# nianticlabs/mickey

Hardware: AMD Instinct MI355X
Metric: image pairs/sec (540x720) (higher is better)
Workload: dtype bf16

## Files before the change

include/mickey_hip.h:

```cpp
#ifndef MICKEY_HIP_H
#define MICKEY_HIP_H

#ifdef __cplusplus
extern "C" {
#endif

typedef void* mk_stream_t;

enum { MK_OK = 0, MK_ERR_INVALID_ARGUMENT = 1, MK_ERR_LAUNCH = 2 };
enum { MK_BF16 = 0, MK_F16 = 1, MK_F32 = 2 };
enum { MK_ACT_NONE = 0, MK_ACT_RELU = 1, MK_ACT_GELU = 2 };
enum { MK_EPI_STORE = 0, MK_EPI_LS_RESIDUAL = 1, MK_EPI_QKV = 2, MK_EPI_PATCH = 3 };

int mk_version(void);
const char* mk_last_error(void);


int mk_preprocess_u8(const unsigned char* src, long long stride_img, int n, int Hs, int Ws, float* dst, int H, int W,
                     mk_stream_t stream);


int mk_gemm(const void* A, int lda, const void* W, int ldw, const float* bias, void* out, int ldc, int M, int N, int K,
            int act, int out_is_f32, int dtype, mk_stream_t stream);

// ... 76 lines not shown
int mk_absmax_scale(const float* x, int d0, int d1, int d2, int d3, long long s0, long long s1, long long s2, long long s3,
                    float* work, float* scale, mk_stream_t stream);

long long mk_conv_train_lead_rows(int Wd);
long long mk_conv_train_plane_rows(int nimg, int H, int Wd);
int mk_conv_train_planes(const float* src, long long stride_b, long long stride_c, long long stride_h, long long stride_w, int nimg,
                         int C, int H, int Wd, const float* scale, void* hi, void* lo, int ld, mk_stream_t stream);

int mk_conv_train_weight_planes(const float* w, int Cout, int Cin, int transposed, const float* w_scale, const float* act_scale,
                                void* planes, float* acc_scale, mk_stream_t stream);

long long mk_conv_wgrad_work_floats(int Cout, int Cin, int nimg, int H, int Wd);
int mk_conv_wgrad(const void* gy_hi, const void* gy_lo, int ldg, const void* x_hi, const void* x_lo, int Cout, int Cin, int nimg, int H,
                  int Wd, const float* gy_scale, const float* x_scale, float* work, float* dw, mk_stream_t stream);

int mk_posenc_add(const void* x, const float* pe, float* xs, void* cat, int ld_cat, int groups, int nimg, int npix, int C,
                  int dtype, mk_stream_t stream);

long long mk_linattn_work_floats(int groups, int nimg, int L, int C);
int mk_linattn_kv(const float* qkv, float* kv, float* work, int groups, int nimg, int L, int C, mk_stream_t stream);
int mk_linattn_apply(const float* qkv, const float* kv, void* out, int ldo, int groups, int nimg, int L, int C, int dtype,
                     mk_stream_t stream);

long long mk_linattn_train_work_floats(int nimg, int L, int S, int C);
int mk_linattn_train_fwd(const float* q, long long ldq, long long sq, const float* k, long long ldk, long long sk, const float* v,
                         long long ldv, long long sv, float eps, float* out, float* kv, float* work, int nimg, int L, int S, int C,
                         mk_stream_t stream);
int mk_linattn_train_bwd(const float* q, long long ldq, long long sq, const float* k, long long ldk, long long sk, const float* v,
                         long long ldv, long long sv, const float* kv, const float* go, float eps, float* work, float* gkv, float* gq,
                         float* gk, float* gv, int nimg, int L, int S, int C, mk_stream_t stream);

int mk_head_tails(const float* feat_det, const float* w_score, const float* feat_off, const float* w_xy,
                  const float* feat_depth, const float* w_depth, const float* feat_dsc, float* scr, float* kps, float* depth,
                  float* dsc, int nimg, int h, int w, int C, int Cd, int border, int use_softmax, int use_depth_sigmoid,
                  float max_depth, int norm_dsc, float down, mk_stream_t stream);


long long mk_dual_softmax_work_floats(int B, int n0, int n1, int own_copy);
int mk_dual_softmax(const float* dsc0, const float* dsc1, const float* scr0, const float* scr1, float inv_temperature,
                    int use_dustbin, float dustbin, float* scores, float* kp_scores, float* final_scores, float* work, int B,
                    int C, int n0, int n1, mk_stream_t stream);

long long mk_dual_softmax_split_work_floats(int B, int n0, int n1);
int mk_dual_softmax_split(const float* dsc0, const float* dsc1, const float* scr0, const float* scr1, float inv_temperature,
                          int use_dustbin, float dustbin, float* scores, float* kp_scores, float* final_scores, float* work,
                          int B, int C, int n0, int n1, mk_stream_t stream);
// ... 87 lines not shown
```

mickey_amd/_native.py:

```python
import ctypes
import os

import torch

from . import build as _build

MK_BF16, MK_F16, MK_F32 = 0, 1, 2
ACT_NONE, ACT_RELU, ACT_GELU = 0, 1, 2

_P, _I, _L, _F, _U = ctypes.c_void_p, ctypes.c_int, ctypes.c_longlong, ctypes.c_float, ctypes.c_ulonglong
_CODES = {"p": _P, "i": _I, "l": _L, "f": _F, "u": _U}

SIGNATURES = {
    "mk_version": ("i", ""),
    "mk_last_error": ("s", ""),
    "mk_preprocess_u8": ("i", "pliiipiip"),
    "mk_gemm": ("i", "pipippiiiiiiip"),
    "mk_gemm_grouped": ("i", "pilpilplpiliiiiiiip"),
    "mk_gemm_ls_residual": ("i", "pipipppiiiiip"),
    "mk_gemm_qkv": ("i", "pipippppiiiifip"),
    "mk_gemm_patch_embed": ("i", "pipipppiiiiip"),
    "mk_gemm_ls_residual_ln": ("i", "pipippppipppiiiiip"),
    "mk_gemm_patch_embed_ln": ("i", "pipipppppiiiiip"),
    "mk_cls_token_ln": ("i", "pppppiiiip"),
# ... 5 lines not shown
    "mk_layernorm": ("i", "pippfpiipiiiiiiiiiip"),
    "mk_layernorm_nchw": ("i", "pippfpiiiiiip"),
    "mk_gemm_ln128": ("i", "pilpilppfpipiiiiiiip"),
    "mk_layernorm_planes": ("i", "pippfppifpiiiiiiiiipp"),
    "mk_flash_attn_fwd": ("i", "ppppiiiiiip"),
    "mk_bordered_rows": ("l", "iii"),
    "mk_conv3x3": ("i", "pliplipilplplpiliiiiiiip"),
    "mk_conv3x3_split": ("i", "pplipplipilplppiliiiiiiffpp"),
    "mk_conv3x3_split_dscale": ("i", "ppipipiiiipp"),
    "mk_split_planes": ("i", "plilfpplpp"),
    "mk_absmax_scale_work_floats": ("l", ""),
    "mk_absmax_scale": ("i", "piiiillllppp"),
    "mk_conv_train_lead_rows": ("l", "i"),
    "mk_conv_train_plane_rows": ("l", "iii"),
    "mk_conv_train_planes": ("i", "plllliiiipppip"),
    "mk_conv_train_weight_planes": ("i", "piiippppp"),
    "mk_conv_wgrad_work_floats": ("l", "iiiii"),
    "mk_conv_wgrad": ("i", "ppippiiiiippppp"),
    "mk_gemm_grouped_split": ("i", "ppilpilplppiliiiiiffpp"),
    "mk_posenc_add": ("i", "ppppiiiiiip"),
    "mk_linattn_work_floats": ("l", "iiii"),
    "mk_linattn_kv": ("i", "pppiiiip"),
    "mk_linattn_apply": ("i", "pppiiiiiip"),
    "mk_linattn_train_work_floats": ("l", "iiii"),
    "mk_linattn_train_fwd": ("i", "pllpllpllfpppiiiip"),
    "mk_linattn_train_bwd": ("i", "pllpllpllppfpppppiiiip"),
    "mk_head_tails": ("i", "pppppppppppiiiiiiiififp"),
    "mk_dual_softmax_work_floats": ("l", "iiii"),
    "mk_dual_softmax": ("i", "ppppfifppppiiiip"),
    "mk_dual_softmax_split_work_floats": ("l", "iii"),
    "mk_dual_softmax_split": ("i", "ppppfifppppiiiip"),
    "mk_sinkhorn_work_floats": ("l", "iii"),
    "mk_sinkhorn": ("i", "ppppfippppiiiip"),
    "mk_dual_softmax_kf": ("i", "ppppfifppppiiiipip"),
    "mk_dual_softmax_split_kf": ("i", "ppppfifppppiiiipip"),
    "mk_sinkhorn_kf": ("i", "ppppfippppiiiipip"),
    "mk_mutual_nn": ("i", "ppppiiip"),
    "mk_dual_softmax_train_work_floats": ("l", "iiii"),
    "mk_dual_softmax_train": ("i", "ppppfppppppiiiiip"),
    "mk_dual_softmax_bwd_work_floats": ("l", "iiii"),
    "mk_dual_softmax_bwd": ("i", "ppppfpppppppppiiiiip"),
    "mk_exprace_topk_work_bytes": ("l", "iiil"),
    "mk_exprace_topk_state_bytes": ("l", "ii"),
    "mk_exprace_topk": ("i", "ppuupppppiiliip"),
    "mk_counter_add": ("i", "pup"),
    "mk_gather_backproject": ("i", "ppppppppppppiiiiip"),
# ... 95 lines not shown
```

mickey_amd/csrc/mk_heads.hip:

```cpp
#include "mk_common.hpp"

namespace {
using namespace mk;

constexpr int KVW = 272;
constexpr int KV_CHUNK = 64;

template <typename T>
__global__ __launch_bounds__(256) void posenc_kernel(const T* __restrict__ x, const float* __restrict__ pe,
                                                     float* __restrict__ xs, T* __restrict__ cat, int ld_cat, long long rows,
                                                     int npix, int C, long long total4) {
  for (long long i = blockIdx.x * (long long)blockDim.x + threadIdx.x; i < total4; i += (long long)gridDim.x * blockDim.x) {
    const int c4 = (int)(i % (C / 4));
    const long long r = i / (C / 4);
    const long long rr = r % rows;
    const int pix = (int)(rr % npix);
    const typename Lp<T>::V4 v = *(const typename Lp<T>::V4*)(x + r * C + c4 * 4);
    f32x4 f;
#pragma unroll
    for (int e = 0; e < 4; ++e) f[e] = (float)v[e];
    if (pe) f += *(const f32x4*)(pe + (long long)pix * C + c4 * 4);
    *(f32x4*)(xs + r * C + c4 * 4) = f;
    typename Lp<T>::V4 o;
#pragma unroll
    for (int e = 0; e < 4; ++e) o[e] = (T)f[e];
    *(typename Lp<T>::V4*)(cat + r * ld_cat + c4 * 4) = o;
  }
}

__device__ __forceinline__ float phi(float x) { return x > 0.f ? x + 1.0f : expf(x); }

__global__ __launch_bounds__(256) void linattn_kv_partial(const float* __restrict__ qkv, float* __restrict__ part, int L, int C,
                                                          int nchunk) {
  extern __shared__ __attribute__((aligned(16))) float skv[];
  const int H = C >> 4;
  const long long gi = blockIdx.y;
  const int chunk = blockIdx.x;
  const int t = threadIdx.x, lane = t & 63, wave = t >> 6;
  const int s0 = chunk * KV_CHUNK, ntok = min(L, s0 + KV_CHUNK) - s0;
  const float invL = 1.0f / (float)L;
  const float* base = qkv + (gi * (long long)L + s0) * 3 * C + C;
  const int c4 = 2 * C / 4;
  for (int it = 0; it < KV_CHUNK * c4 / 256; ++it) {
    const int i = it * 256 + t;
    const int s = min(i / c4, ntok - 1), c = (i % c4) * 4;
    glds16(base + (long long)s * 3 * C + c, (char*)skv + (it * 256 + wave * 64) * 16);
  }
  asm volatile("s_waitcnt vmcnt(0)" ::: "memory");
  __syncthreads();
  for (int i = t; i < ntok * (C / 4); i += 256) {
    const int s = i / (C / 4), c = (i - s * (C / 4)) * 4;
    f32x4 v = *(const f32x4*)(skv + s * 2 * C + c);
#pragma unroll
    for (int e = 0; e < 4; ++e) v[e] = phi(v[e]);
    *(f32x4*)(skv + s * 2 * C + c) = v;
  }
  __syncthreads();
  const int h = lane >> 3, vh = (lane >> 2) & 1, dg = lane & 3;
  float acc[4][8];
  float ks[4] = {0.f, 0.f, 0.f, 0.f};
#pragma unroll
  for (int a = 0; a < 4; ++a)
#pragma unroll
    for (int e = 0; e < 8; ++e) acc[a][e] = 0.f;
  if (h < H) {
    for (int s = wave; s < ntok; s += 4) {
      const float* row = skv + s * 2 * C + h * 16;
      const f32x4 k4 = *(const f32x4*)(row + dg * 4);
      const f32x4 v0 = *(const f32x4*)(row + C + vh * 8), v1 = *(const f32x4*)(row + C + vh * 8 + 4);
#pragma unroll
      for (int a = 0; a < 4; ++a) {
#pragma unroll
        for (int e = 0; e < 4; ++e) {
          acc[a][e] += k4[a] * (v0[e] * invL);
          acc[a][4 + e] += k4[a] * (v1[e] * invL);
        }
        ks[a] += k4[a];
      }
    }
  }
  __syncthreads();
  if (h < H) {
    float* o = skv + (wave * H + h) * KVW;
#pragma unroll
    for (int a = 0; a < 4; ++a) {
#pragma unroll
      for (int e = 0; e < 8; ++e) o[(dg * 4 + a) * 16 + vh * 8 + e] = acc[a][e];
      if (vh == 0) o[256 + dg * 4 + a] = ks[a];
    }
  }
  __syncthreads();
  for (int i = t; i < H * KVW; i += 256) {
    const int hh = i / KVW, e = i - hh * KVW;
    const float r = ((skv[(0 * H + hh) * KVW + e] + skv[(1 * H + hh) * KVW + e]) + skv[(2 * H + hh) * KVW + e]) + skv[(3 * H + hh) * KVW + e];
    part[(((gi * H + hh) * nchunk) + chunk) * KVW + e] = r;
  }
}

__global__ __launch_bounds__(KVW) void linattn_kv_reduce(const float* __restrict__ part, float* __restrict__ kv, int nchunk) {
  const long long gih = blockIdx.x;
  const int t = threadIdx.x;
// ... 3 lines not shown
}

template <typename T>
__global__ __launch_bounds__(256) void linattn_apply_kernel(const float* __restrict__ qkv, const float* __restrict__ kv,
                                                            T* __restrict__ out, int ldo, int L, int C) {
  extern __shared__ __attribute__((aligned(16))) float skv[];
  const int H = C >> 4;
  const long long gi = blockIdx.y;
  for (int i = threadIdx.x; i < H * KVW; i += blockDim.x) skv[(i / KVW) * 273 + (i % KVW)] = kv[gi * H * KVW + i];
  __syncthreads();
  const int tpb = 256 / H;
  const int h = threadIdx.x % H;
  const int s = blockIdx.x * tpb + threadIdx.x / H;
  if (s >= L || threadIdx.x >= tpb * H) return;
  const float* qrow = qkv + (gi * L + s) * 3 * C + h * 16;
  float Q[16];
#pragma unroll
  for (int d4 = 0; d4 < 4; ++d4) {
    const f32x4 t4 = *(const f32x4*)(qrow + d4 * 4);
#pragma unroll
    for (int e = 0; e < 4; ++e) Q[d4 * 4 + e] = phi(t4[e]);
  }
  const float* K = skv + h * 273;
  float z = 0.f;
#pragma unroll
  for (int d = 0; d < 16; ++d) z += Q[d] * K[256 + d];
  const float scale = (float)L / (z + 1e-6f);
  typename Lp<T>::V8 o0, o1;
#pragma unroll
  for (int v = 0; v < 16; ++v) {
    float a = 0.f;
#pragma unroll
    for (int d = 0; d < 16; ++d) a += Q[d] * K[d * 16 + v];
    a *= scale;
    if (v < 8) o0[v] = (T)a; else o1[v - 8] = (T)a;
  }
  T* orow = out + (gi * L + s) * ldo + h * 16;
  *(typename Lp<T>::V8*)orow = o0;
  *(typename Lp<T>::V8*)(orow + 8) = o1;
}


__global__ __launch_bounds__(256) void kp_depth_tail_kernel(const float* __restrict__ fdet, const float* __restrict__ wsc,
                                                            const float* __restrict__ foff, const float* __restrict__ wxy,
                                                            const float* __restrict__ fdep, const float* __restrict__ wd,
                                                            float* __restrict__ scr, float* __restrict__ kps,
                                                            float* __restrict__ depth, int nimg, int h, int w, int C,
                                                            int use_depth_sigmoid, float max_depth, float down) {
  const int n = h * w;
  const long long gp = blockIdx.x * 4LL + (threadIdx.x >> 6);
  if (gp >= (long long)nimg * n) return;
  const int lane = threadIdx.x & 63;
  const int img = (int)(gp / n), p = (int)(gp % n);
  float as = 0.f, ax = 0.f, ay = 0.f, ad = 0.f;
  for (int c = lane; c < C; c += 64) {
    const float fo = foff[gp * C + c];
    as += fdet[gp * C + c] * wsc[c];
    ax += fo * wxy[c];
    ay += fo * wxy[C + c];
// ... 56 lines not shown

__global__ __launch_bounds__(256) void dsc_tail_kernel(const float* __restrict__ fdsc, float* __restrict__ dsc, int n, int Cd,
                                                       int norm_dsc) {
  extern __shared__ __attribute__((aligned(16))) float tile[];
  const int img = blockIdx.y, p0 = blockIdx.x * 64;
  const int lane = threadIdx.x & 63, wave = threadIdx.x >> 6;
  for (int pp = wave; pp < 64; pp += 4) {
    const int p = p0 + pp;
    if (p >= n) break;
    const float* f = fdsc + ((long long)img * n + p) * Cd;
    float q = 0.f;
    for (int c = lane; c < Cd; c += 64) q += f[c] * f[c];
    q = wave_sum(q);
    const float sc = norm_dsc ? 1.0f / sqrtf(q + 1e-10f) : 1.0f;
    for (int c = lane; c < Cd; c += 64) tile[c * 65 + pp] = f[c] * sc;
  }
  __syncthreads();
  for (int i = threadIdx.x; i < Cd * 64; i += blockDim.x) {
    const int c = i >> 6, pp = i & 63;
    if (p0 + pp < n) dsc[((long long)img * Cd + c) * n + p0 + pp] = tile[c * 65 + pp];
  }
}

template <typename T>
__global__ __launch_bounds__(256, 2) void gemm_ln128_kernel(const T* __restrict__ A, int lda, long long strideA, const T* __restrict__ W,
                                                            int ldw, long long strideW, const float* __restrict__ lnw,
                                                            const float* __restrict__ lnb, float eps, float* __restrict__ resid, int ldr,
                                                            T* __restrict__ out, int ldo, int groups, int M, int K, int bord_h, int bord_w) {
  using V8 = typename Lp<T>::V8;
  using V4 = typename Lp<T>::V4;
  extern __shared__ __attribute__((aligned(16))) char smem[];
  const int lane = threadIdx.x & 63, wave = threadIdx.x >> 6;
  const int g = blockIdx.x % groups, wg = blockIdx.x / groups, nwg = gridDim.x / groups;
  const int ks = K >> 5;
  const T* Wg = W + (long long)g * strideW;
  for (int i = threadIdx.x; i < 128 * ks * 4; i += 256) {
    const int c = i & 3, s = (i >> 2) % ks, n = i / (4 * ks);
    const uint4 v = *(const uint4*)(Wg + (long long)n * ldw + s * 32 + c * 8);
    *(uint4*)(smem + ((s * 128 + n) * 64 + ((c ^ ((n >> 2) & 3)) << 4))) = v;
  }
  float* slw = (float*)(smem + 128 * K * 2);
  float* slb = slw + 128;
  if (threadIdx.x < 128) {
    slw[threadIdx.x] = lnw[g * 128 + threadIdx.x];
    slb[threadIdx.x] = lnb[g * 128 + threadIdx.x];
  }
// ... 19 lines not shown
  };
  if (wg < ntile) {
    load_x(wg);
    if (resid) load_r(wg);
  }
  for (int tile = wg; tile < ntile; tile += nwg) {
    const int row = row_of(tile);
    const bool ok = row < M;
    const bool more = tile + nwg < ntile;
    f32x4 acc[8];
#pragma unroll
    for (int f = 0; f < 8; ++f) acc[f] = f32x4{0.f, 0.f, 0.f, 0.f};
#pragma unroll
    for (int s = 0; s < 8; ++s) {
      if (s >= ks) break;
#pragma unroll
      for (int f = 0; f < 8; ++f) {
        const int n = f * 16 + r16;
        const V8 wf = *(const V8*)(smem + ((s * 128 + n) * 64 + ((q ^ ((n >> 2) & 3)) << 4)));
        acc[f] = Lp<T>::mma16(wf, xf[s], acc[f]);
      }
    }
    if (more) load_x(tile + nwg);
    float sm = 0.f;
#pragma unroll
    for (int f = 0; f < 8; ++f) sm += (acc[f][0] + acc[f][1]) + (acc[f][2] + acc[f][3]);
    sm += __shfl_xor(sm, 16, 64);
    sm += __shfl_xor(sm, 32, 64);
    const float mean = sm * (1.0f / 128.0f);
    float qs = 0.f;
#pragma unroll
    for (int f = 0; f < 8; ++f) {
#pragma unroll
      for (int e = 0; e < 4; ++e) {
        acc[f][e] -= mean;
        qs += acc[f][e] * acc[f][e];
      }
    }
    qs += __shfl_xor(qs, 16, 64);
    qs += __shfl_xor(qs, 32, 64);
    const float rstd = 1.0f / sqrtf(qs * (1.0f / 128.0f) + eps);
    if (ok) {
      const long long grow = (long long)g * M + row;
      const long long orow = bord_h > 0 ? (long long)g * brows + bordered_row(row, bord_h, bord_w) : grow;
#pragma unroll
      for (int f = 0; f < 8; ++f) {
        const int fe = f * 16 + q * 4;
        const f32x4 ww = *(const f32x4*)(slw + fe), bb = *(const f32x4*)(slb + fe);
        f32x4 y;
#pragma unroll
        for (int e = 0; e < 4; ++e) y[e] = acc[f][e] * rstd * ww[e] + bb[e];
        if (resid) {
          y += rv[f];
          *(f32x4*)(resid + grow * ldr + fe) = y;
        }
        V4 o;
#pragma unroll
        for (int e = 0; e < 4; ++e) o[e] = (T)y[e];
        *(V4*)(out + orow * ldo + fe) = o;
      }
    }
    if (resid && more) load_r(tile + nwg);
  }
}

}

extern "C" {

int mk_posenc_add(const void* x, const float* pe, float* xs, void* cat, int ld_cat, int groups, int nimg, int npix, int C,
                  int dtype, mk_stream_t stream) {
  MK_CHECK_ARG(x && xs && cat && groups > 0 && nimg > 0 && npix > 0 && C % 8 == 0 && ld_cat % 4 == 0 && ld_cat >= C,
               "mk_posenc_add: bad args");
  const long long rows = (long long)nimg * npix;
  const long long total4 = (long long)groups * rows * (C / 4);
  int blocks = (int)((total4 + 255) / 256);
  if (blocks > 8192) blocks = 8192;
  if (dtype == MK_BF16)
    hipLaunchKernelGGL(posenc_kernel<__bf16>, dim3(blocks), dim3(256), 0, (hipStream_t)stream, (const __bf16*)x, pe, xs,
                       (__bf16*)cat, ld_cat, rows, npix, C, total4);
  else if (dtype == MK_F16)
    hipLaunchKernelGGL(posenc_kernel<_Float16>, dim3(blocks), dim3(256), 0, (hipStream_t)stream, (const _Float16*)x, pe, xs,
                       (_Float16*)cat, ld_cat, rows, npix, C, total4);
  else
    hipLaunchKernelGGL(posenc_kernel<float>, dim3(blocks), dim3(256), 0, (hipStream_t)stream, (const float*)x, pe, xs,
                       (float*)cat, ld_cat, rows, npix, C, total4);
// ... 16 lines not shown
                     nchunk);
  MK_CHECK_LAUNCH();
  hipLaunchKernelGGL(linattn_kv_reduce, dim3(gih), dim3(KVW), 0, (hipStream_t)stream, work, kv, nchunk);
  MK_CHECK_LAUNCH();
  return MK_OK;
}

int mk_linattn_apply(const float* qkv, const float* kv, void* out, int ldo, int groups, int nimg, int L, int C, int dtype,
                     mk_stream_t stream) {
  const int H = C / 16;
  MK_CHECK_ARG(qkv && kv && out && groups > 0 && nimg > 0 && L > 0 && C % 16 == 0 && H <= 64 && ldo % 8 == 0 && ldo >= C,
               "mk_linattn_apply: bad args");
  const int tpb = 256 / H;
  dim3 grid((L + tpb - 1) / tpb, groups * nimg);
  const size_t lds = (size_t)H * 273 * sizeof(float);
  if (dtype == MK_BF16)
    hipLaunchKernelGGL(linattn_apply_kernel<__bf16>, grid, dim3(256), lds, (hipStream_t)stream, qkv, kv, (__bf16*)out, ldo, L,
                       C);
  else if (dtype == MK_F16)
    hipLaunchKernelGGL(linattn_apply_kernel<_Float16>, grid, dim3(256), lds, (hipStream_t)stream, qkv, kv, (_Float16*)out,
                       ldo, L, C);
  else
    hipLaunchKernelGGL(linattn_apply_kernel<float>, grid, dim3(256), lds, (hipStream_t)stream, qkv, kv, (float*)out, ldo, L, C);
  MK_CHECK_LAUNCH();
  return MK_OK;
}

int mk_gemm_ln128(const void* A, int lda, long long strideA, const void* W, int ldw, long long strideW, const float* ln_w,
                  const float* ln_b, float eps, float* resid, int ldr, void* out, int ldo, int groups, int M, int K, int bord_h,
                  int bord_w, int dtype, mk_stream_t stream) {
  MK_CHECK_ARG(A && W && ln_w && ln_b && out, "mk_gemm_ln128: null pointer");
  MK_CHECK_ARG(dtype == MK_BF16 || dtype == MK_F16, "mk_gemm_ln128: 16-bit operands only");
  MK_CHECK_ARG(groups > 0 && M > 0 && K >= 32 && K <= 256 && K % 32 == 0 && lda % 8 == 0 && lda >= K && ldw % 8 == 0 && ldw >= K &&
                   ldo % 4 == 0 && ldo >= 128 && (!resid || (ldr % 4 == 0 && ldr >= 128)),
               "mk_gemm_ln128: bad geometry (K a multiple of 32 up to 256, 128 output features)");
  MK_CHECK_ARG((((uintptr_t)A | (uintptr_t)W) & 15) == 0 && ((uintptr_t)out & 7) == 0 && (strideA % 8) == 0 && (strideW % 8) == 0,
               "mk_gemm_ln128: operands must be 16-byte aligned");
  MK_CHECK_ARG(bord_h == 0 || (bord_w > 0 && M % (bord_h * bord_w) == 0), "mk_gemm_ln128: bordered output needs M = nimg * bord_h * bord_w");
  const int lds = 128 * K * 2 + 1024;
  const int ntile = (M + 63) / 64;
  int per_group = ((K > 128 ? 2 : 3) * mk::gemm::num_cus() + groups - 1) / groups;
  if (per_group > ntile) per_group = ntile;
  const dim3 grid((unsigned)(per_group * groups));
  hipError_t e = hipSuccess;
  if (dtype == MK_BF16) {
    static bool done = false;
// ... 39 lines not shown
```

mickey_amd/ops.py:

```python

import numpy as np
import torch


from ._native import ACT_GELU, ACT_NONE, ACT_RELU, call, dtype_code, ptr, query, stream

LOG2E = 1.4426950408889634


def _chk(t, dtype=None):
    assert t.is_cuda and t.is_contiguous(), "expected a contiguous device tensor"
    if dtype is not None:
        assert t.dtype == dtype, "expected %s, got %s" % (dtype, t.dtype)
    return t


def preprocess_u8(frames, H, W, out=None):
    assert frames.is_cuda and frames.dtype == torch.uint8 and frames.dim() == 4 and frames.shape[3] == 3 and frames.is_contiguous()
    n, Hs, Ws, _ = frames.shape
    if out is None:
        out = torch.empty((n, 3, H, W), device=frames.device, dtype=torch.float32)
    call("mk_preprocess_u8", ptr(frames), Hs * Ws * 3, n, Hs, Ws, ptr(out), H, W, stream())
    return out

# ... 295 lines not shown
        dw = torch.empty((Cout, Cin, 3, 3), device=xp[0].device, dtype=torch.float32)
    assert dw.dtype == torch.float32 and dw.is_contiguous() and tuple(dw.shape) == (Cout, Cin, 3, 3)
    work = torch.empty(max(1, int(query("mk_conv_wgrad_work_floats", Cout, Cin, nimg, H, W))), device=dw.device, dtype=torch.float32)
    call("mk_conv_wgrad", ptr(gy[0]), ptr(gy[1]), ldg, ptr(xp[0]), ptr(xp[1]), Cout, Cin, nimg, H, W, ptr(gy_scale), ptr(x_scale),
         ptr(work), ptr(dw), stream())
    return dw


def posenc_add(x, pe, xs, cat, groups, nimg, npix, C):
    call("mk_posenc_add", ptr(x), ptr(pe), ptr(xs), ptr(cat), cat.stride(-2), groups, nimg, npix, C, dtype_code(x.dtype),
         stream())


def linattn_work_floats(groups, nimg, L, C):
    return query("mk_linattn_work_floats", groups, nimg, L, C)


def linattn_kv(qkv, kv, work, groups, nimg, L, C):
    call("mk_linattn_kv", ptr(qkv), ptr(kv), ptr(work), groups, nimg, L, C, stream())


def linattn_apply(qkv, kv, out, ldo, groups, nimg, L, C):
    call("mk_linattn_apply", ptr(qkv), ptr(kv), ptr(out), ldo, groups, nimg, L, C, dtype_code(out.dtype), stream())


def _attn_rows(t):
    N, T, H, D = t.shape
    assert t.dtype == torch.float32 and D == 16 and t.stride(3) == 1 and (H == 1 or t.stride(2) == 16)
    ld = t.stride(1) if T > 1 else H * 16
    return ptr(t), ld, t.stride(0) if N > 1 else T * ld


def linattn_train_fwd(q, k, v, eps):
    N, L, H, _ = q.shape
    S, C = k.shape[1], H * 16
    out = torch.empty((N, L, H, 16), device=q.device, dtype=torch.float32)
    kv = torch.empty((N * H, 272), device=q.device, dtype=torch.float32)
    work = torch.empty(int(query("mk_linattn_train_work_floats", N, L, S, C)), device=q.device, dtype=torch.float32)
    call("mk_linattn_train_fwd", *_attn_rows(q), *_attn_rows(k), *_attn_rows(v), float(eps), ptr(out), ptr(kv), ptr(work), N, L, S, C,
         stream())
    return out, kv


def linattn_train_bwd(q, k, v, kv, go, eps, need):
    N, L, H, _ = q.shape
    S, C = k.shape[1], H * 16
# ... 330 lines not shown
```

mickey_amd/pipeline.py:

```python
import torch

from . import ops
from . import weights as wts_mod


class Workspace:

    def __init__(self):
        self.bufs = {}
        self.sat_flag = None

    def get_planes(self, name, shape, device, zero=False):
        t = self.get(name, (2,) + tuple(shape), torch.float16, device, zero=zero)
        return t[0], t[1]

    def get(self, name, shape, dtype, device, zero=False):
        key = (name, tuple(shape), dtype)
        t = self.bufs.get(key)
        if t is None or t.device != device:
            t = (torch.zeros if zero else torch.empty)(tuple(shape), dtype=dtype, device=device)
            self.bufs[key] = t
        return t


# ... 113 lines not shown
                              stride_in1=R * co, stride_in2=s_in, stride_w=rb.w2.shape[1] * rb.w2.shape[2], stride_bias=co,
                              stride_out=(M if last else R) * co, out_bordered=not last)
            if not last:
                xp = xo
        else:
            h1 = ws.get("rb%d_h" % bi + geo, (G, R, co), lp, dev, zero=True)
            xo = ws.get("rb%d_x" % bi + geo, (G, M if last else R, co), lp, dev, zero=not last)
            ops.conv3x3(x_in, c_in, rb.w1, rb.b1, h1, co, G, nimg, gh, gw, act=ops.ACT_RELU, stride_in1=s_in,
                        stride_w=rb.w1.shape[1] * rb.w1.shape[2], stride_bias=co, stride_out=R * co, out_bordered=True)
            ops.conv3x3(h1, co, rb.w2, rb.b2, xo, co, G, nimg, gh, gw, act=ops.ACT_RELU, in2=x_in, C2=c_in,
                        stride_in1=R * co, stride_in2=s_in, stride_w=rb.w2.shape[1] * rb.w2.shape[2], stride_bias=co,
                        stride_out=(M if last else R) * co, out_bordered=not last)
        x_in, c_in, s_in = xo, co, R * co
    C = c_in
    xs = ws.get("att_xs", (G, M, C), torch.float32, dev)
    cat = ws.get("att_cat", (G, M, 2 * C), lp, dev)
    pe = wts_mod.sine_pos_table(W, C, gh, gw, dev)
    kp_pe, dsc_pe = bool(mk["KP_HEADS"]["POS_ENCODING"]), bool(mk["DSC_HEAD"]["POS_ENCODING"])
    if kp_pe == dsc_pe:
        ops.posenc_add(x_in, pe if kp_pe else None, xs, cat, G, nimg, n, C)
    else:
        ops.posenc_add(x_in[:3], pe if kp_pe else None, xs[:3], cat[:3], 3, nimg, n, C)
        ops.posenc_add(x_in[3:], pe if dsc_pe else None, xs[3:], cat[3:], 1, nimg, n, C)
    qkv = ws.get("att_qkv", (G, M, 3 * C), torch.float32, dev)
    kv = ws.get("att_kv", (G * nimg * (C // 16), 272), torch.float32, dev)
    kvw = ws.get("att_kvw", (ops.linattn_work_floats(G, nimg, n, C),), torch.float32, dev)
    msg = ws.get("att_msg", (G, M, C), lp, dev)
    mrg = ws.get("att_mrg", (G, M, C), torch.float32, dev)
    hid = ws.get("att_hid", (G, M, 2 * C), lp, dev)
    if split:
        x4 = None
        x4h, x4l = plane_pair("att_out", (G, R, C))
    else:
        x4 = ws.get("att_out" + geo, (G, R, C), lp, dev, zero=True)
    nl = len(W.att)
    if split:
        catp = ws.get_planes("att_cat_hl", (G, M, 2 * C), dev)
        msgp = ws.get_planes("att_msg_hl", (G, M, C), dev)
        hidp = ws.get_planes("att_hid_hl", (G, M, 2 * C), dev)
    for li, lay in enumerate(W.att):
        last = li == nl - 1
        if split:
            if li == 0:
                ops.split_planes(cat[:, :, :C], catp[0][:, :, :C], catp[1][:, :, :C], sat=sat)
            ops.gemm_grouped_split(catp, lay.qkv_w, None, qkv, G, M, 3 * C, C, 2 * C, 3 * C, M * 2 * C, 3 * C * 2 * C, 0, M * 3 * C,
                                   w_scale=wsc(lay.qkv_w), sat=sat)
            ops.linattn_kv(qkv, kv, kvw, G, nimg, n, C)
            ops.linattn_apply(qkv, kv, msg, C, G, nimg, n, C)
            ops.split_planes(msg, msgp[0], msgp[1], sat=sat)
            ops.gemm_grouped_split(msgp, lay.merge_w, None, mrg, G, M, C, C, C, C, M * C, C * 2 * C, 0, M * C, w_scale=wsc(lay.merge_w), sat=sat)
            ops.layernorm(mrg, lay.n1w, lay.n1b, 1e-5, out=(catp[0][:, :, C:], catp[1][:, :, C:]), ldo=2 * C, rows_out=G * M,
                          rows_per_img=G * M, wgroup_rows=M, sat=sat)
            ops.gemm_grouped_split(catp, lay.mlp0_w, None, hidp, G, M, 2 * C, 2 * C, 2 * C, 2 * C, M * 2 * C, 2 * C * 2 * 2 * C, 0,
                                   M * 2 * C, act=ops.ACT_RELU, w_scale=wsc(lay.mlp0_w), sat=sat)
            ops.gemm_grouped_split(hidp, lay.mlp2_w, None, mrg, G, M, C, 2 * C, 2 * C, C, M * 2 * C, C * 2 * 2 * C, 0, M * C,
                                   w_scale=wsc(lay.mlp2_w), sat=sat)
        else:
            ops.gemm_grouped(cat, lay.qkv_w, None, qkv, G, M, 3 * C, C, 2 * C, C, 3 * C, M * 2 * C, 3 * C * C, 0, M * 3 * C)
            ops.linattn_kv(qkv, kv, kvw, G, nimg, n, C)
            ops.linattn_apply(qkv, kv, msg, C, G, nimg, n, C)
            fused_ln = C == 128 and lp != torch.float32
            if fused_ln:
                ops.gemm_ln128(msg, lay.merge_w, lay.n1w, lay.n1b, 1e-5, cat[:, :, C:], G, M, C, ldo=2 * C)
            else:
                ops.gemm_grouped(msg, lay.merge_w, None, mrg, G, M, C, C, C, C, C, M * C, C * C, 0, M * C)
                ops.layernorm(mrg, lay.n1w, lay.n1b, 1e-5, out=cat[:, :, C:], ldo=2 * C, rows_out=G * M, rows_per_img=G * M,
                              wgroup_rows=M)
            ops.gemm_grouped(cat, lay.mlp0_w, None, hid, G, M, 2 * C, 2 * C, 2 * C, 2 * C, 2 * C, M * 2 * C, 4 * C * C, 0,
                             M * 2 * C, act=ops.ACT_RELU)
            if not fused_ln:
                ops.gemm_grouped(hid, lay.mlp2_w, None, mrg, G, M, C, 2 * C, 2 * C, 2 * C, C, M * 2 * C, 2 * C * C, 0, M * C)
        if split:
            o2 = (x4h, x4l) if last else (catp[0][:, :, :C], catp[1][:, :, :C])
        else:
            o2 = x4 if last else cat
        if not split and C == 128 and lp != torch.float32:
            ops.gemm_ln128(hid, lay.mlp2_w, lay.n2w, lay.n2b, 1e-5, o2, G, M, 2 * C, ldo=C if last else 2 * C, resid=xs,
                           bordered=(nimg, gh, gw) if last else None)
        else:
# ... 104 lines not shown
```

Before: 274.5.

## Fuse QKV projection into linear-attention KV and apply kernels with merge+LayerNorm

Adds two fused kernels for C=128 bf16/f16. One computes the K/V projections with MFMA directly from the concatenated input and accumulates the per-chunk KV outer products. The other recomputes Q, applies attention, then runs the merge GEMM and LayerNorm in the same kernel, writing straight into the concat buffer. This removes the fp32 qkv tensor, the intermediate message buffer and separate launches, at the cost of recomputing projections in both kernels and needing large LDS with more register pressure. It is enabled by default for the non-split low-precision path.

New measurement: 277.4 (median of 6 runs). 1.01x the previous value.

```diff
diff --git a/include/mickey_hip.h b/include/mickey_hip.h
--- a/include/mickey_hip.h
+++ b/include/mickey_hip.h
@@ -122,6 +122,13 @@
 int mk_linattn_apply(const float* qkv, const float* kv, void* out, int ldo, int groups, int nimg, int L, int C, int dtype,
                      mk_stream_t stream);
 
+int mk_linattn_kv_fused(const void* x, int lda, long long strideX, const void* qkv_w, int ldw, long long strideW, float* kv,
+                        float* work, int groups, int nimg, int L, int C, int dtype, mk_stream_t stream);
+int mk_linattn_apply_fused(const void* x, int lda, long long strideX, const void* qkv_w, int ldw, long long strideW, const float* kv,
+                           const void* merge_w, int ldwm, long long strideWm, const float* ln_w, const float* ln_b, float eps,
+                           void* out, int ldo, long long strideOut, int groups, int nimg, int L, int C, int dtype,
+                           mk_stream_t stream);
+
 long long mk_linattn_train_work_floats(int nimg, int L, int S, int C);
 int mk_linattn_train_fwd(const float* q, long long ldq, long long sq, const float* k, long long ldk, long long sk, const float* v,
                          long long ldv, long long sv, float eps, float* out, float* kv, float* work, int nimg, int L, int S, int C,
diff --git a/mickey_amd/_native.py b/mickey_amd/_native.py
--- a/mickey_amd/_native.py
+++ b/mickey_amd/_native.py
@@ -51,6 +51,8 @@
     "mk_linattn_work_floats": ("l", "iiii"),
     "mk_linattn_kv": ("i", "pppiiiip"),
     "mk_linattn_apply": ("i", "pppiiiiiip"),
+    "mk_linattn_kv_fused": ("i", "pilpilppiiiiip"),
+    "mk_linattn_apply_fused": ("i", "pilpilppilppfpiliiiiip"),
     "mk_linattn_train_work_floats": ("l", "iiii"),
     "mk_linattn_train_fwd": ("i", "pllpllpllfpppiiiip"),
     "mk_linattn_train_bwd": ("i", "pllpllpllppfpppppiiiip"),
diff --git a/mickey_amd/csrc/mk_heads.hip b/mickey_amd/csrc/mk_heads.hip
--- a/mickey_amd/csrc/mk_heads.hip
+++ b/mickey_amd/csrc/mk_heads.hip
@@ -29,6 +29,32 @@
 }
 
 __device__ __forceinline__ float phi(float x) { return x > 0.f ? x + 1.0f : expf(x); }
+
+template <int NV>
+__device__ __forceinline__ void kv_outer(float (&acc)[4][NV], float (&ks)[4], const f32x4 k4, const float (&vs)[NV]) {
+#pragma unroll
+  for (int a = 0; a < 4; ++a) {
+#pragma unroll
+    for (int e = 0; e < NV; ++e) acc[a][e] += k4[a] * vs[e];
+    ks[a] += k4[a];
+  }
+}
+
+template <int NV, typename KVAT, typename KSAT, typename PUT>
+__device__ __forceinline__ void linattn_apply_cols(const float (&Q)[16], KVAT kvat, KSAT ksat, const int L, PUT put) {
+  float z = 0.f;
+#pragma unroll
+  for (int d = 0; d < 16; ++d) z += Q[d] * ksat(d);
+  const float scale = (float)L / (z + 1e-6f);
+#pragma unroll
+  for (int v = 0; v < NV; ++v) {
+    float s = 0.f;
+#pragma unroll
+    for (int d = 0; d < 16; ++d) s += Q[d] * kvat(d, v);
+    s *= scale;
+    put(v, s);
+  }
+}
 
 __global__ __launch_bounds__(256) void linattn_kv_partial(const float* __restrict__ qkv, float* __restrict__ part, int L, int C,
                                                           int nchunk) {
@@ -68,15 +94,8 @@
       const float* row = skv + s * 2 * C + h * 16;
       const f32x4 k4 = *(const f32x4*)(row + dg * 4);
       const f32x4 v0 = *(const f32x4*)(row + C + vh * 8), v1 = *(const f32x4*)(row + C + vh * 8 + 4);
-#pragma unroll
-      for (int a = 0; a < 4; ++a) {
-#pragma unroll
-        for (int e = 0; e < 4; ++e) {
-          acc[a][e] += k4[a] * (v0[e] * invL);
-          acc[a][4 + e] += k4[a] * (v1[e] * invL);
-        }
-        ks[a] += k4[a];
-      }
+      const float v8[8] = {v0[0] * invL, v0[1] * invL, v0[2] * invL, v0[3] * invL, v1[0] * invL, v1[1] * invL, v1[2] * invL, v1[3] * invL};
+      kv_outer<8>(acc, ks, k4, v8);
     }
   }
   __syncthreads();
@@ -126,19 +145,9 @@
     for (int e = 0; e < 4; ++e) Q[d4 * 4 + e] = phi(t4[e]);
   }
   const float* K = skv + h * 273;
-  float z = 0.f;
-#pragma unroll
-  for (int d = 0; d < 16; ++d) z += Q[d] * K[256 + d];
-  const float scale = (float)L / (z + 1e-6f);
   typename Lp<T>::V8 o0, o1;
-#pragma unroll
-  for (int v = 0; v < 16; ++v) {
-    float a = 0.f;
-#pragma unroll
-    for (int d = 0; d < 16; ++d) a += Q[d] * K[d * 16 + v];
-    a *= scale;
-    if (v < 8) o0[v] = (T)a; else o1[v - 8] = (T)a;
-  }
+  linattn_apply_cols<16>(Q, [&](int d, int v) { return K[d * 16 + v]; }, [&](int d) { return K[256 + d]; }, L,
+                         [&](int v, float a) { if (v < 8) o0[v] = (T)a; else o1[v - 8] = (T)a; });
   T* orow = out + (gi * L + s) * ldo + h * 16;
   *(typename Lp<T>::V8*)orow = o0;
   *(typename Lp<T>::V8*)(orow + 8) = o1;
@@ -241,6 +250,33 @@
   }
 }
 
+__device__ __forceinline__ float ln128_centre(f32x4 (&acc)[8], const float eps) {
+  float sm = 0.f;
+#pragma unroll
+  for (int f = 0; f < 8; ++f) sm += (acc[f][0] + acc[f][1]) + (acc[f][2] + acc[f][3]);
+  sm += __shfl_xor(sm, 16, 64);
+  sm += __shfl_xor(sm, 32, 64);
+  const float mean = sm * (1.0f / 128.0f);
+  float qs = 0.f;
+#pragma unroll
+  for (int f = 0; f < 8; ++f) {
+#pragma unroll
+    for (int e = 0; e < 4; ++e) {
+      acc[f][e] -= mean;
+      qs += acc[f][e] * acc[f][e];
+    }
+  }
+  qs += __shfl_xor(qs, 16, 64);
+  qs += __shfl_xor(qs, 32, 64);
+  return 1.0f / sqrtf(qs * (1.0f / 128.0f) + eps);
+}
+__device__ __forceinline__ f32x4 ln128_affine(const f32x4 c, const float rstd, const f32x4 ww, const f32x4 bb) {
+  f32x4 y;
+#pragma unroll
+  for (int e = 0; e < 4; ++e) y[e] = c[e] * rstd * ww[e] + bb[e];
+  return y;
+}
+
 template <typename T>
 __global__ __launch_bounds__(256, 2) void gemm_ln128_kernel(const T* __restrict__ A, int lda, long long strideA, const T* __restrict__ W,
                                                             int ldw, long long strideW, const float* __restrict__ lnw,
@@ -306,24 +342,7 @@
       }
     }
     if (more) load_x(tile + nwg);
-    float sm = 0.f;
-#pragma unroll
-    for (int f = 0; f < 8; ++f) sm += (acc[f][0] + acc[f][1]) + (acc[f][2] + acc[f][3]);
-    sm += __shfl_xor(sm, 16, 64);
-    sm += __shfl_xor(sm, 32, 64);
-    const float mean = sm * (1.0f / 128.0f);
-    float qs = 0.f;
-#pragma unroll
-    for (int f = 0; f < 8; ++f) {
-#pragma unroll
-      for (int e = 0; e < 4; ++e) {
-        acc[f][e] -= mean;
-        qs += acc[f][e] * acc[f][e];
-      }
-    }
-    qs += __shfl_xor(qs, 16, 64);
-    qs += __shfl_xor(qs, 32, 64);
-    const float rstd = 1.0f / sqrtf(qs * (1.0f / 128.0f) + eps);
+    const float rstd = ln128_centre(acc, eps);
     if (ok) {
       const long long grow = (long long)g * M + row;
       const long long orow = bord_h > 0 ? (long long)g * brows + bordered_row(row, bord_h, bord_w) : grow;
@@ -331,9 +350,7 @@
       for (int f = 0; f < 8; ++f) {
         const int fe = f * 16 + q * 4;
         const f32x4 ww = *(const f32x4*)(slw + fe), bb = *(const f32x4*)(slb + fe);
-        f32x4 y;
-#pragma unroll
-        for (int e = 0; e < 4; ++e) y[e] = acc[f][e] * rstd * ww[e] + bb[e];
+        f32x4 y = ln128_affine(acc[f], rstd, ww, bb);
         if (resid) {
           y += rv[f];
           *(f32x4*)(resid + grow * ldr + fe) = y;
@@ -346,6 +363,258 @@
     }
     if (resid && more) load_r(tile + nwg);
   }
+}
+
+constexpr int FC = 128;
+
+template <typename T, int ROWS>
+__device__ __forceinline__ void w_rows_to_lds(const T* __restrict__ Wg, const int ldw, char* dst, const int tid, const int nthr) {
+  for (int i = tid; i < ROWS * 16; i += nthr) {
+    const int c = i & 3, st = (i >> 2) & 3, n = i >> 4;
+    const uint4 v = *(const uint4*)(Wg + (long long)n * ldw + st * 32 + c * 8);
+    *(uint4*)(dst + ((st * ROWS + n) * 64 + ((c ^ ((n >> 2) & 3)) << 4))) = v;
+  }
+}
+template <typename T, int ROWS>
+__device__ __forceinline__ typename Lp<T>::V8 w_frag(const char* w, const int st, const int n, const int q) {
+  return *(const typename Lp<T>::V8*)(w + ((st * ROWS + n) * 64 + ((q ^ ((n >> 2) & 3)) << 4)));
+}
+
+template <typename T>
+__global__ __launch_bounds__(256, 2) void linattn_kv_fused_kernel(const T* __restrict__ X, int lda, long long strideX,
+                                                                  const T* __restrict__ Wqkv, int ldw, long long strideW,
+                                                                  float* __restrict__ part, int nimg, int L, int nchunk) {
+  using V8 = typename Lp<T>::V8;
+  __shared__ __attribute__((aligned(16))) float stage[4 * 1024];
+  constexpr int H = FC / 16;
+  const int tid = threadIdx.x, lane = tid & 63, wave = __builtin_amdgcn_readfirstlane(tid >> 6);
+  const long long gi = blockIdx.y;
+  const int g = (int)(gi / nimg), img = (int)(gi % nimg);
+  float* stg = stage + wave * 1024;
+  const int r16 = lane & 15, q = lane >> 4;
+  const int hp = lane >> 5, vg = (lane >> 2) & 7, dg = lane & 3;
+  const float invL = 1.0f / (float)L;
+  V8 wf[4][4];
+  {
+    const T* Wg = Wqkv + (long long)g * strideW + q * 8;
+#pragma unroll
+    for (int j = 0; j < 4; ++j) {
+      const int n = FC + (j >> 1) * FC + wave * 32 + (j & 1) * 16 + r16;
+#pragma unroll
+      for (int st = 0; st < 4; ++st) wf[st][j] = *(const V8*)(Wg + (long long)n * ldw + st * 32);
+    }
+  }
+  const T* xi = X + (long long)g * strideX + (long long)img * L * lda + q * 8;
+  auto load_x = [&](int first, V8(&xf)[4]) {
+    const int s = min(first + 4 * r16, L - 1);
+#pragma unroll
+    for (int st = 0; st < 4; ++st) xf[st] = *(const V8*)(xi + (long long)s * lda + st * 32);
+  };
+  V8 xf[4], xn[4];
+  int chunk = blockIdx.x;
+  if (chunk < nchunk) load_x(chunk * KV_CHUNK, xf);
+  for (; chunk < nchunk; chunk += gridDim.x) {
+    const int ntok = min(L, (chunk + 1) * KV_CHUNK) - chunk * KV_CHUNK;
+    float acc[4][4][2], ks[4][4];
+#pragma unroll
+    for (int b = 0; b < 4; ++b)
+#pragma unroll
+      for (int a = 0; a < 4; ++a) acc[b][a][0] = acc[b][a][1] = ks[b][a] = 0.f;
+#pragma unroll
+    for (int b = 0; b < 4; ++b) {
+      f32x4 kvq[4];
+#pragma unroll
+      for (int j = 0; j < 4; ++j) kvq[j] = f32x4{0.f, 0.f, 0.f, 0.f};
+#pragma unroll
+      for (int st = 0; st < 4; ++st)
+#pragma unroll
+        for (int j = 0; j < 4; ++j) kvq[j] = Lp<T>::mma16(wf[st][j], xf[st], kvq[j]);
+#pragma unroll
+      for (int st = 0; st < 4; ++st) xn[st] = xf[st];
+      if (b < 3) load_x(chunk * KV_CHUNK + b + 1, xn);
+      else if (chunk + (int)gridDim.x < nchunk) load_x((chunk + gridDim.x) * KV_CHUNK, xn);
+#pragma unroll
+      for (int j = 0; j < 2; ++j)
+#pragma unroll
+        for (int e = 0; e < 4; ++e) {
+          kvq[j][e] = phi(kvq[j][e]);
+          kvq[2 + j][e] = kvq[2 + j][e] * invL;
+        }
+#pragma unroll
+      for (int j = 0; j < 4; ++j) *(f32x4*)(stg + r16 * 64 + (((j * 4 + q) ^ r16) << 2)) = kvq[j];
+      __builtin_amdgcn_wave_barrier();
+      auto token = [&](const int t) {
+        const f32x4 k4 = *(const f32x4*)(stg + t * 64 + (((hp * 4 + dg) ^ t) << 2));
+        const float2 v2 = *(const float2*)(stg + t * 64 + (((8 + hp * 4 + (vg >> 1)) ^ t) << 2) + (vg & 1) * 2);
+        const float vs[2] = {v2.x, v2.y};
+        kv_outer<2>(acc[b], ks[b], k4, vs);
+      };
+      if (ntok == KV_CHUNK) {
+#pragma unroll
+        for (int t = 0; t < 16; ++t) token(t);
+      } else {
+#pragma unroll 1
+        for (int t = 0; b + 4 * t < ntok; ++t) token(t);
+      }
+      __builtin_amdgcn_wave_barrier();
+#pragma unroll
+      for (int st = 0; st < 4; ++st) xf[st] = xn[st];
+    }
+    float* o = part + (((gi * H + 2 * wave + hp) * nchunk) + chunk) * KVW;
+#pragma unroll
+    for (int a = 0; a < 4; ++a) {
+      float2 r;
+      r.x = ((acc[0][a][0] + acc[1][a][0]) + acc[2][a][0]) + acc[3][a][0];
+      r.y = ((acc[0][a][1] + acc[1][a][1]) + acc[2][a][1]) + acc[3][a][1];
+      *(float2*)(o + (dg * 4 + a) * 16 + vg * 2) = r;
+    }
+    if (vg == 0) {
+      f32x4 r;
+#pragma unroll
+      for (int a = 0; a < 4; ++a) r[a] = ((ks[0][a] + ks[1][a]) + ks[2][a]) + ks[3][a];
+      *(f32x4*)(o + 256 + dg * 4) = r;
+    }
+  }
+}
+
+template <typename T, bool MERGE>
+__global__ __launch_bounds__(512) void linattn_apply_fused_kernel(const T* X, int lda, long long strideX, const T* __restrict__ Wqkv,
+                                                                  int ldw, long long strideW, const float* __restrict__ kv,
+                                                                  const T* __restrict__ Wm, int ldwm, long long strideWm,
+                                                                  const float* __restrict__ lnw, const float* __restrict__ lnb, float eps,
+                                                                  T* out, int ldo, long long strideO, int nimg, int L) {
+  using V8 = typename Lp<T>::V8;
+  using V4 = typename Lp<T>::V4;
+  extern __shared__ __attribute__((aligned(16))) char smem[];
+  constexpr int H = FC / 16;
+  const int tid = threadIdx.x, lane = tid & 63, wave = __builtin_amdgcn_readfirstlane(tid >> 6);
+  const long long gi = blockIdx.y;
+  const int g = (int)(gi / nimg), img = (int)(gi % nimg);
+  char* swm = smem + FC * FC * 2;
+  float* slw = (float*)(smem + 2 * FC * FC * 2);
+  float* slb = slw + FC;
+  w_rows_to_lds<T, FC>(Wqkv + (long long)g * strideW, ldw, smem, tid, 512);
+  if (MERGE) {
+    w_rows_to_lds<T, FC>(Wm + (long long)g * strideWm, ldwm, swm, tid, 512);
+    if (tid < FC) {
+      slw[tid] = lnw[g * FC + tid];
+      slb[tid] = lnb[g * FC + tid];
+    }
+  }
+  __syncthreads();
+  float* stq = (float*)(smem + 2 * FC * FC * 2 + 1024) + wave * 2048;
+  const int r16 = lane & 15, q = lane >> 4;
+  const int par = lane >> 5, h = (lane >> 2) & 7, vg = lane & 3;
+  f32x4 kreg[16], ksum[4];
+  {
+    const float* kp = kv + (gi * H + h) * KVW;
+#pragma unroll
+    for (int d = 0; d < 16; ++d) kreg[d] = *(const f32x4*)(kp + d * 16 + vg * 4);
+#pragma unroll
+    for (int d4 = 0; d4 < 4; ++d4) ksum[d4] = *(const f32x4*)(kp + 256 + d4 * 4);
+  }
+  const int ntile = (L + 15) >> 4, step = gridDim.x * 8;
+  const T* xi = X + (long long)g * strideX + (long long)img * L * lda + q * 8;
+  T* oi = out + (long long)g * strideO + (long long)img * L * ldo;
+  V8 xf[4];
+  auto load_x = [&](int tile) {
+    const int s = min(tile * 16 + r16, L - 1);
+#pragma unroll
+    for (int st = 0; st < 4; ++st) xf[st] = *(const V8*)(xi + (long long)s * lda + st * 32);
+  };
+  int tile = blockIdx.x * 8 + wave;
+  if (tile < ntile) load_x(tile);
+  for (; tile < ntile; tile += step) {
+    f32x4 acc[8];
+#pragma unroll
+    for (int f = 0; f < 8; ++f) acc[f] = f32x4{0.f, 0.f, 0.f, 0.f};
+#pragma unroll
+    for (int st = 0; st < 4; ++st)
+#pragma unroll
+      for (int f = 0; f < 8; ++f) acc[f] = Lp<T>::mma16(w_frag<T, FC>(smem, st, f * 16 + r16, q), xf[st], acc[f]);
+    if (tile + step < ntile) load_x(tile + step);
+#pragma unroll
+    for (int f = 0; f < 8; ++f) {
+#pragma unroll
+      for (int e = 0; e < 4; ++e) acc[f][e] = phi(acc[f][e]);
+      const int c = f * 4 + q;
+      *(f32x4*)(stq + r16 * 128 + ((c ^ r16 ^ ((c >> 4) << 1)) << 2)) = acc[f];
+    }
+    __builtin_amdgcn_wave_barrier();
+    V4 msg[8];
+#pragma unroll
+    for (int i = 0; i < 8; ++i) {
+      const int t = 2 * i + par;
+      float Q[16];
+#pragma unroll
+      for (int d4 = 0; d4 < 4; ++d4) {
+        const int c = h * 4 + d4;
+        const f32x4 t4 = *(const f32x4*)(stq + t * 128 + ((c ^ t ^ ((c >> 4) << 1)) << 2));
+#pragma unroll
+        for (int e = 0; e < 4; ++e) Q[d4 * 4 + e] = t4[e];
+      }
+      linattn_apply_cols<4>(Q, [&](int d, int v) { return kreg[d][v]; }, [&](int d) { return ksum[d >> 2][d & 3]; }, L,
+                            [&](int v, float a) { msg[i][v] = (T)a; });
+      if constexpr (!MERGE) {
+        const int s = tile * 16 + t;
+        if (s < L) *(V4*)(oi + (long long)s * ldo + h * 16 + vg * 4) = msg[i];
+      }
+    }
+    if constexpr (MERGE) {
+      __builtin_amdgcn_wave_barrier();
+      char* stm = (char*)stq;
+#pragma unroll
+      for (int i = 0; i < 8; ++i) {
+        const int t = 2 * i + par;
+        *(V4*)(stm + t * 256 + (((h * 2 + (vg >> 1)) ^ t) << 4) + (vg & 1) * 8) = msg[i];
+      }
+      __builtin_amdgcn_wave_barrier();
+      V8 mf[4];
+#pragma unroll
+      for (int st = 0; st < 4; ++st) mf[st] = *(const V8*)(stm + r16 * 256 + (((st * 4 + q) ^ r16) << 4));
+      __builtin_amdgcn_wave_barrier();
+#pragma unroll
+      for (int f = 0; f < 8; ++f) acc[f] = f32x4{0.f, 0.f, 0.f, 0.f};
+#pragma unroll
+      for (int st = 0; st < 4; ++st)
+#pragma unroll
+        for (int f = 0; f < 8; ++f) acc[f] = Lp<T>::mma16(w_frag<T, FC>(swm, st, f * 16 + r16, q), mf[st], acc[f]);
+      const float rstd = ln128_centre(acc, eps);
+      const int s = tile * 16 + r16;
+      if (s < L) {
+#pragma unroll
+        for (int f = 0; f < 8; ++f) {
+          const int fe = f * 16 + q * 4;
+          const f32x4 y = ln128_affine(acc[f], rstd, *(const f32x4*)(slw + fe), *(const f32x4*)(slb + fe));
+          V4 o;
+#pragma unroll
+          for (int e = 0; e < 4; ++e) o[e] = (T)y[e];
+          *(V4*)(oi + (long long)s * ldo + fe) = o;
+        }
+      }
+    }
+  }
+}
+
+template <typename T>
+hipError_t launch_apply_fused(bool merge, dim3 grid, int lds, hipStream_t st, const void* x, int lda, long long strideX,
+                                     const void* qkv_w, int ldw, long long strideW, const float* kv, const void* merge_w, int ldwm,
+                                     long long strideWm, const float* ln_w, const float* ln_b, float eps, void* out, int ldo,
+                                     long long strideOut, int nimg, int L) {
+  static bool done[2] = {false, false};
+  const void* fn = merge ? (const void*)linattn_apply_fused_kernel<T, true> : (const void*)linattn_apply_fused_kernel<T, false>;
+  if (!done[merge]) {
+    const hipError_t e = hipFuncSetAttribute(fn, hipFuncAttributeMaxDynamicSharedMemorySize, lds);
+    if (e != hipSuccess) return e;
+    done[merge] = true;
+  }
+  if (merge)
+    hipLaunchKernelGGL((linattn_apply_fused_kernel<T, true>), grid, dim3(512), lds, st, (const T*)x, lda, strideX, (const T*)qkv_w, ldw,
+                       strideW, kv, (const T*)merge_w, ldwm, strideWm, ln_w, ln_b, eps, (T*)out, ldo, strideOut, nimg, L);
+  else
+    hipLaunchKernelGGL((linattn_apply_fused_kernel<T, false>), grid, dim3(512), lds, st, (const T*)x, lda, strideX, (const T*)qkv_w, ldw,
+                       strideW, kv, (const T*)merge_w, ldwm, strideWm, ln_w, ln_b, eps, (T*)out, ldo, strideOut, nimg, L);
+  return hipSuccess;
 }
 
 }
@@ -408,6 +677,57 @@
                        ldo, L, C);
   else
     hipLaunchKernelGGL(linattn_apply_kernel<float>, grid, dim3(256), lds, (hipStream_t)stream, qkv, kv, (float*)out, ldo, L, C);
+  MK_CHECK_LAUNCH();
+  return MK_OK;
+}
+
+int mk_linattn_kv_fused(const void* x, int lda, long long strideX, const void* qkv_w, int ldw, long long strideW, float* kv,
+                        float* work, int groups, int nimg, int L, int C, int dtype, mk_stream_t stream) {
+  MK_CHECK_ARG(x && qkv_w && kv && work, "mk_linattn_kv_fused: null pointer");
+  MK_CHECK_ARG(C == FC && (dtype == MK_BF16 || dtype == MK_F16), "mk_linattn_kv_fused: C = 128 and 16-bit operands only");
+  MK_CHECK_ARG(groups > 0 && nimg > 0 && L > 0 && lda % 8 == 0 && lda >= C && ldw % 8 == 0 && ldw >= C && strideX % 8 == 0 &&
+                   strideW % 8 == 0 && (((uintptr_t)x | (uintptr_t)qkv_w | (uintptr_t)work) & 15) == 0,
+               "mk_linattn_kv_fused: bad geometry (rows of 8-element multiples, 16-byte aligned)");
+  const int nchunk = (L + KV_CHUNK - 1) / KV_CHUNK;
+  const int gi = groups * nimg;
+  int per_img = (8 * mk::gemm::num_cus() + gi - 1) / gi;
+  if (per_img > nchunk) per_img = nchunk;
+  if (dtype == MK_BF16)
+    hipLaunchKernelGGL(linattn_kv_fused_kernel<__bf16>, dim3(per_img, gi), dim3(256), 0, (hipStream_t)stream, (const __bf16*)x, lda,
+                       strideX, (const __bf16*)qkv_w, ldw, strideW, work, nimg, L, nchunk);
+  else
+    hipLaunchKernelGGL(linattn_kv_fused_kernel<_Float16>, dim3(per_img, gi), dim3(256), 0, (hipStream_t)stream, (const _Float16*)x,
+                       lda, strideX, (const _Float16*)qkv_w, ldw, strideW, work, nimg, L, nchunk);
+  MK_CHECK_LAUNCH();
+  hipLaunchKernelGGL(linattn_kv_reduce, dim3(gi * (C / 16)), dim3(KVW), 0, (hipStream_t)stream, work, kv, nchunk);
+  MK_CHECK_LAUNCH();
+  return MK_OK;
+}
+
+int mk_linattn_apply_fused(const void* x, int lda, long long strideX, const void* qkv_w, int ldw, long long strideW, const float* kv,
+                           const void* merge_w, int ldwm, long long strideWm, const float* ln_w, const float* ln_b, float eps,
+                           void* out, int ldo, long long strideOut, int groups, int nimg, int L, int C, int dtype,
+                           mk_stream_t stream) {
+  MK_CHECK_ARG(x && qkv_w && kv && out, "mk_linattn_apply_fused: null pointer");
+  MK_CHECK_ARG(C == FC && (dtype == MK_BF16 || dtype == MK_F16), "mk_linattn_apply_fused: C = 128 and 16-bit operands only");
+  MK_CHECK_ARG(!merge_w || (ln_w && ln_b && ldwm % 8 == 0 && ldwm >= C && strideWm % 8 == 0 && ((uintptr_t)merge_w & 15) == 0),
+               "mk_linattn_apply_fused: merge_w comes with ln_w, ln_b and 16-byte aligned rows");
+  MK_CHECK_ARG(groups > 0 && nimg > 0 && L > 0 && lda % 8 == 0 && lda >= C && ldw % 8 == 0 && ldw >= C && ldo % 4 == 0 && ldo >= C &&
+                   strideX % 8 == 0 && strideW % 8 == 0 && strideOut % 4 == 0 && (((uintptr_t)x | (uintptr_t)qkv_w | (uintptr_t)kv) & 15) == 0 &&
+                   ((uintptr_t)out & 7) == 0,
+               "mk_linattn_apply_fused: bad geometry (rows of 8-element multiples, 16-byte aligned; out 8-byte aligned)");
+  const int ntile = (L + 127) / 128;
+  const int gi = groups * nimg;
+  int per_img = (mk::gemm::num_cus() + gi - 1) / gi;
+  if (per_img > ntile) per_img = ntile;
+  const int lds = 2 * FC * FC * 2 + 1024 + 8 * 8192;
+  const dim3 grid(per_img, gi);
+  const hipError_t e = dtype == MK_BF16
+      ? launch_apply_fused<__bf16>(merge_w != nullptr, grid, lds, (hipStream_t)stream, x, lda, strideX, qkv_w, ldw, strideW, kv, merge_w,
+                                   ldwm, strideWm, ln_w, ln_b, eps, out, ldo, strideOut, nimg, L)
+      : launch_apply_fused<_Float16>(merge_w != nullptr, grid, lds, (hipStream_t)stream, x, lda, strideX, qkv_w, ldw, strideW, kv, merge_w,
+                                     ldwm, strideWm, ln_w, ln_b, eps, out, ldo, strideOut, nimg, L);
+  if (e != hipSuccess) { mk_set_error("mk_linattn_apply_fused: cannot reserve %d B of LDS: %s", lds, hipGetErrorString(e)); return MK_ERR_LAUNCH; }
   MK_CHECK_LAUNCH();
   return MK_OK;
 }
diff --git a/mickey_amd/ops.py b/mickey_amd/ops.py
--- a/mickey_amd/ops.py
+++ b/mickey_amd/ops.py
@@ -341,6 +341,21 @@
 
 def linattn_apply(qkv, kv, out, ldo, groups, nimg, L, C):
     call("mk_linattn_apply", ptr(qkv), ptr(kv), ptr(out), ldo, groups, nimg, L, C, dtype_code(out.dtype), stream())
+
+
+def linattn_kv_fused(x, qkv_w, kv, work, groups, nimg, L, C, lda=None):
+    lda = x.stride(-2) if lda is None else lda
+    call("mk_linattn_kv_fused", ptr(x), lda, x.stride(0), ptr(qkv_w), qkv_w.stride(-2), qkv_w.stride(0), ptr(kv), ptr(work), groups, nimg,
+         L, C, dtype_code(x.dtype), stream())
+
+
+def linattn_apply_fused(x, qkv_w, kv, out, groups, nimg, L, C, merge_w=None, ln_w=None, ln_b=None, eps=1e-5, lda=None):
+    lda = x.stride(-2) if lda is None else lda
+    mw = merge_w is not None
+    call("mk_linattn_apply_fused", ptr(x), lda, x.stride(0), ptr(qkv_w), qkv_w.stride(-2), qkv_w.stride(0), ptr(kv), ptr(merge_w),
+         merge_w.stride(-2) if mw else 0, merge_w.stride(0) if mw else 0, ptr(ln_w), ptr(ln_b), float(eps), ptr(out), out.stride(-2),
+         out.stride(0), groups, nimg, L, C, dtype_code(x.dtype), stream())
+    return out
 
 
 def _attn_rows(t):
diff --git a/mickey_amd/pipeline.py b/mickey_amd/pipeline.py
--- a/mickey_amd/pipeline.py
+++ b/mickey_amd/pipeline.py
@@ -159,10 +159,12 @@
     else:
         ops.posenc_add(x_in[:3], pe if kp_pe else None, xs[:3], cat[:3], 3, nimg, n, C)
         ops.posenc_add(x_in[3:], pe if dsc_pe else None, xs[3:], cat[3:], 1, nimg, n, C)
-    qkv = ws.get("att_qkv", (G, M, 3 * C), torch.float32, dev)
+    fused_att = bool(cfg["AMD"].get("LINATTN_FUSED", True)) and not split and C == 128 and lp != torch.float32
     kv = ws.get("att_kv", (G * nimg * (C // 16), 272), torch.float32, dev)
     kvw = ws.get("att_kvw", (ops.linattn_work_floats(G, nimg, n, C),), torch.float32, dev)
-    msg = ws.get("att_msg", (G, M, C), lp, dev)
+    if not fused_att:
+        qkv = ws.get("att_qkv", (G, M, 3 * C), torch.float32, dev)
+        msg = ws.get("att_msg", (G, M, C), lp, dev)
     mrg = ws.get("att_mrg", (G, M, C), torch.float32, dev)
     hid = ws.get("att_hid", (G, M, 2 * C), lp, dev)
     if split:
@@ -192,6 +194,11 @@
                                    M * 2 * C, act=ops.ACT_RELU, w_scale=wsc(lay.mlp0_w), sat=sat)
             ops.gemm_grouped_split(hidp, lay.mlp2_w, None, mrg, G, M, C, 2 * C, 2 * C, C, M * 2 * C, C * 2 * 2 * C, 0, M * C,
                                    w_scale=wsc(lay.mlp2_w), sat=sat)
+        elif fused_att:
+            ops.linattn_kv_fused(cat, lay.qkv_w, kv, kvw, G, nimg, n, C)
+            ops.linattn_apply_fused(cat, lay.qkv_w, kv, cat[:, :, C:], G, nimg, n, C, merge_w=lay.merge_w, ln_w=lay.n1w, ln_b=lay.n1b)
+            ops.gemm_grouped(cat, lay.mlp0_w, None, hid, G, M, 2 * C, 2 * C, 2 * C, 2 * C, 2 * C, M * 2 * C, 4 * C * C, 0,
+                             M * 2 * C, act=ops.ACT_RELU)
         else:
             ops.gemm_grouped(cat, lay.qkv_w, None, qkv, G, M, 3 * C, C, 2 * C, C, 3 * C, M * 2 * C, 3 * C * C, 0, M * 3 * C)
             ops.linattn_kv(qkv, kv, kvw, G, nimg, n, C)
```
